# santurini/vsrlab

Hardware: AMD Instinct MI355X
Metric: LR frames/sec fwd+bwd, BasicVSR 4x 540p 7-frame clip, 1->8 MI355X (higher is better)
Workload: dtype bf16; 1 GPU; BasicVSR(mid=64,res_blocks=30,x4) fwd+Charbonnier+bwd+clip+Adam, 540x960->2160x3840, 7-frame clip, 2 clips per GPU (BASELINE configs[1]); clips_per_gpu=2, frames=7, res_blocks=30, parallelism=single GPU, arena=full, train_flow=False, trunk_chains=True

## Files before the change

### include/vsrlab_hip.h

```cpp
#ifndef VSRLAB_HIP_H
#define VSRLAB_HIP_H
#include <stddef.h>
#ifdef __cplusplus
extern "C" {
#endif

#define VSR_DT_F32 0
#define VSR_DT_BF16 1

#define VSR_STATUS_OK 0
#define VSR_STATUS_BADARG (-1)
#define VSR_STATUS_UNSUPPORTED (-2)
#define VSR_STATUS_HIP (-3)
#define VSR_STATUS_WORKSPACE (-4)

int vsr_abi_version(void);
const char* vsr_status_string(int status);

typedef struct VsrBasicVSRDesc {
    int n, t, h, w;
    int mid_channels;
    int res_blocks;
    int upscale;
    int dtype;
// ... 59 lines not shown

int vsr_flow_warp_fwd_ex(int dtype, const void* in_pm, const float* flow, void* out_pm, int N, int H, int W, int C,
                         int padding_mode, void* stream);
int vsr_flow_warp_bwd_ex(int dtype, const void* dout_pm, const float* flow, float* dacc_pm_f32, int N, int H, int W, int C,
                         int padding_mode, void* stream);
int vsr_flow_warp_bwd_flow_ex(int dtype, const void* in_pm, const void* dout_pm, const float* flow, float* dflow, int N,
                              int H, int W, int C, int padding_mode, void* stream);

int vsr_planar_to_pm(int dtype, const float* in, void* out_pm, int N, int Cin, int H, int W, int C,
                     void* stream);
int vsr_pm_to_planar(int dtype, const void* in_pm, float* out, int N, int Cout, int H, int W, int C,
                     void* stream);

int vsr_conv3x3_c64_fwd(int dtype, const void* x_pm, const float* w, const float* b, void* wpack,
                        void* y_pm, const void* res_pm, int act, int N, int H, int W, void* stream);

size_t vsr_conv3x3_c64_chain_sync_bytes(int nlayers, int N, int H, int W);
int vsr_conv3x3_c64_chain_fwd(const void* images, const void* wpack, const float* bias, int nlayers, int N, int H, int W,
                              void* sync, void* stream);
int vsr_conv3x3_c64_dgrad(int dtype, const void* dy_pm, const float* w, void* wpack, void* dx_pm,
                          const void* res_pm, const void* aux_pm, int mask_mode, int N, int H,
                          int W, void* stream);
int vsr_conv_layer_fwd(int dtype, int ks, const void* x_pm, int cin_pm, const float* lr_planar, const float* w,
                       const float* b, int cin_real, int cout_real, void* wpack, void* y_pm, int cd, float* y_planar,
                       int act, float slope, int pixel_shuffle, int N, int H, int W, void* stream);
size_t vsr_conv_layer_bwd_scratch_bytes(int dtype, int N, int H, int W, int pixel_shuffle);
int vsr_conv_layer_bwd(int dtype, int ks, const void* x_pm, int cin_pm, const float* lr_planar, const float* w, int cin_real,
                       int cout_real, const void* y_pm, const float* y_planar, const void* dy_pm, const float* dy_planar, int cd,
                       int act, float slope, int pixel_shuffle, void* dx_pm, float* dlr_planar, float* gw, float* gb,
                       void* scratch, size_t scratch_bytes, int N, int H, int W, void* stream);
size_t vsr_conv3x3_c64_wgrad_slab_floats(void);
int vsr_conv3x3_c64_wgrad(int dtype, const void* x_pm, const void* dy_pm, float* gw, float* gb,
                          float* slab, int N, int H, int W, void* stream);

size_t vsr_charbonnier_scratch_floats(void);
int vsr_charbonnier_fwd_bwd(const float* sr, const float* hr, float* dsr, float* loss, float* scratch, long long numel,
                            float eps, void* stream);

size_t vsr_optim_scratch_floats(void);
int vsr_adam_clip_step(float* params, const float* grads, float* exp_avg, float* exp_avg_sq, long long numel,
                       float lr, float beta1, float beta2, float eps, float weight_decay, int step, float grad_scale,
                       float max_norm, float* scratch, float* norm_out, void* stream);
int vsr_grad_norm(const float* grads, long long numel, float grad_scale, float* scratch, float* norm_out, void* stream);

int vsr_resize_bilinear(const float* in, float* out, long long planes, int H, int W, int h, int w, void* stream);

typedef struct VsrDiscDesc { int n, h, w, mid_ch, dtype; } VsrDiscDesc;
size_t vsr_disc_workspace_bytes(const VsrDiscDesc* d, int need_backward);
int vsr_disc_forward(const VsrDiscDesc* d, const float* const* params, int nparams, const float* img, float* out,
                     void* workspace, size_t workspace_bytes, int need_backward, void* stream);
int vsr_disc_backward(const VsrDiscDesc* d, float* const* grads, int nparams, const float* img, const float* dout,
                      float* dimg, void* workspace, size_t workspace_bytes, void* stream);

int vsr_spectral_norm(const float* w_orig, float* u, float* v, float* w_out, float* sigma, int rows, int cols,
                      int training, void* stream);
#define VSR_SN_SCRATCH_FLOATS 1024
int vsr_spectral_norm_backward(const float* dw, const float* w_orig, const float* u, const float* v, const float* sigma,
                               float* dw_orig, int rows, int cols, float* scratch, void* stream);

int vsr_bce_with_logits(const float* x, float target, float* dx, float* loss, long long numel, void* stream);

typedef struct VsrAttnDesc {
    int B, N, heads, head_dim;
    int q0, k0, o0, Nq, Nk;
    int Cout, c_off;
    int nW, Nm;
// ... 18 lines not shown
```

### vsrlab_amd/_lib.py

```python
import ctypes
import os
from ctypes import c_char_p, c_float, c_int, c_longlong, c_size_t, c_void_p

_HERE = os.path.dirname(os.path.abspath(__file__))
LIB_PATH = os.environ.get("VSRLAB_AMD_LIB") or os.path.join(_HERE, "lib", "libvsrlab_hip.so")

DT_F32 = 0
DT_BF16 = 1


class BasicVSRDesc(ctypes.Structure):
    _fields_ = [("n", c_int), ("t", c_int), ("h", c_int), ("w", c_int), ("mid_channels", c_int),
                ("res_blocks", c_int), ("upscale", c_int), ("dtype", c_int), ("arena_mode", c_int)]


class DiscDesc(ctypes.Structure):
    _fields_ = [("n", c_int), ("h", c_int), ("w", c_int), ("mid_ch", c_int), ("dtype", c_int)]


class AttnDesc(ctypes.Structure):
    _fields_ = [(k, c_int) for k in ("B", "N", "heads", "head_dim", "q0", "k0", "o0", "Nq", "Nk", "Cout", "c_off", "nW", "Nm")] + \
               [("scale", c_float), ("dtype", c_int), ("mask_packed", c_int), ("mask_value", c_float)]


# ... 7 lines not shown
    "vsr_basicvsr_backward": (c_int, [ctypes.POINTER(BasicVSRDesc), _P, _P, c_int, _P, _P, _P, _P, c_size_t, _P]),
    "vsr_basicvsr_get_flows": (c_int, [ctypes.POINTER(BasicVSRDesc), _P, _P, _P, _P]),
    "vsr_basicvsr_narrow_workspace_bytes": (c_size_t, [ctypes.POINTER(BasicVSRDesc), c_int]),
    "vsr_basicvsr_narrow_forward": (c_int, [ctypes.POINTER(BasicVSRDesc), _P, c_int, _P, _P, _P, c_size_t, c_int, _P]),
    "vsr_basicvsr_narrow_backward": (c_int, [ctypes.POINTER(BasicVSRDesc), _P, _P, c_int, _P, _P, _P, _P, c_size_t, _P]),
    "vsr_basicvsr_narrow_get_flows": (c_int, [ctypes.POINTER(BasicVSRDesc), _P, _P, _P, _P]),
    "vsr_spynet_workspace_bytes": (c_size_t, [c_int, c_int, c_int, c_int, c_int]),
    "vsr_spynet_forward": (c_int, [c_int, c_int, c_int, c_int, _P, c_int, _P, _P, _P, _P, c_size_t, c_int, _P]),
    "vsr_spynet_backward": (c_int, [c_int, c_int, c_int, c_int, _P, c_int, _P, _P, c_size_t, _P]),
    "vsr_spynet_forward_ex": (c_int, [c_int, c_int, c_int, c_int, _P, c_int, _P, _P, c_int, _P, _P, c_size_t, c_int, _P]),
    "vsr_spynet_backward_ex": (c_int, [c_int, c_int, c_int, c_int, _P, _P, c_int, _P, c_int, _P, _P, _P, _P, c_size_t, _P]),
    "vsr_cleaner_workspace_bytes": (c_size_t, [c_int, c_int, c_int, c_int, c_int, c_int, c_int]),
    "vsr_cleaner_narrow_workspace_bytes": (c_size_t, [c_int, c_int, c_int, c_int, c_int, c_int, c_int, c_int]),
    "vsr_cleaner_forward": (c_int, [c_int, c_int, c_int, c_int, c_int, c_int, c_int, _P, c_int, _P, _P, _P, c_size_t, c_int, _P]),
    "vsr_cleaner_backward": (c_int, [c_int, c_int, c_int, c_int, c_int, c_int, c_int, _P, c_int, _P, _P, _P, _P, c_size_t, _P]),
    "vsr_flow_warp_fwd": (c_int, [c_int, _P, _P, _P, c_int, c_int, c_int, c_int, _P]),
    "vsr_flow_warp_bwd": (c_int, [c_int, _P, _P, _P, c_int, c_int, c_int, c_int, _P]),
    "vsr_flow_warp_bwd_flow": (c_int, [c_int, _P, _P, _P, _P, c_int, c_int, c_int, c_int, _P]),
    "vsr_flow_warp_fwd_ex": (c_int, [c_int, _P, _P, _P, c_int, c_int, c_int, c_int, c_int, _P]),
    "vsr_flow_warp_bwd_ex": (c_int, [c_int, _P, _P, _P, c_int, c_int, c_int, c_int, c_int, _P]),
    "vsr_flow_warp_bwd_flow_ex": (c_int, [c_int, _P, _P, _P, _P, c_int, c_int, c_int, c_int, c_int, _P]),
    "vsr_planar_to_pm": (c_int, [c_int, _P, _P, c_int, c_int, c_int, c_int, c_int, _P]),
    "vsr_pm_to_planar": (c_int, [c_int, _P, _P, c_int, c_int, c_int, c_int, c_int, _P]),
    "vsr_conv3x3_c64_fwd": (c_int, [c_int, _P, _P, _P, _P, _P, _P, c_int, c_int, c_int, c_int, _P]),
    "vsr_conv3x3_c64_chain_sync_bytes": (c_size_t, [c_int, c_int, c_int, c_int]),
    "vsr_conv3x3_c64_chain_fwd": (c_int, [_P, _P, _P, c_int, c_int, c_int, c_int, _P, _P]),
    "vsr_conv3x3_c64_dgrad": (c_int, [c_int, _P, _P, _P, _P, _P, _P, c_int, c_int, c_int, c_int, _P]),
    "vsr_conv_layer_fwd": (c_int, [c_int, c_int, _P, c_int, _P, _P, _P, c_int, c_int, _P, _P, c_int, _P, c_int, c_float, c_int, c_int, c_int, c_int, _P]),
    "vsr_conv_layer_bwd_scratch_bytes": (c_size_t, [c_int, c_int, c_int, c_int, c_int]),
    "vsr_conv_layer_bwd": (c_int, [c_int, c_int, _P, c_int, _P, _P, c_int, c_int, _P, _P, _P, _P, c_int, c_int, c_float, c_int, _P, _P, _P, _P,
                                   _P, c_size_t, c_int, c_int, c_int, _P]),
    "vsr_conv3x3_c64_wgrad_slab_floats": (c_size_t, []),
    "vsr_conv3x3_c64_wgrad": (c_int, [c_int, _P, _P, _P, _P, _P, c_int, c_int, c_int, _P]),
    "vsr_charbonnier_scratch_floats": (c_size_t, []),
    "vsr_charbonnier_fwd_bwd": (c_int, [_P, _P, _P, _P, _P, c_longlong, c_float, _P]),
    "vsr_optim_scratch_floats": (c_size_t, []),
    "vsr_adam_clip_step": (c_int, [_P, _P, _P, _P, c_longlong, c_float, c_float, c_float, c_float, c_float, c_int, c_float,
                                   c_float, _P, _P, _P]),
    "vsr_grad_norm": (c_int, [_P, c_longlong, c_float, _P, _P, _P]),
    "vsr_resize_bilinear": (c_int, [_P, _P, c_longlong, c_int, c_int, c_int, c_int, _P]),
    "vsr_disc_workspace_bytes": (c_size_t, [ctypes.POINTER(DiscDesc), c_int]),
    "vsr_disc_forward": (c_int, [ctypes.POINTER(DiscDesc), _P, c_int, _P, _P, _P, c_size_t, c_int, _P]),
    "vsr_disc_backward": (c_int, [ctypes.POINTER(DiscDesc), _P, c_int, _P, _P, _P, _P, c_size_t, _P]),
    "vsr_spectral_norm": (c_int, [_P, _P, _P, _P, _P, c_int, c_int, c_int, _P]),
    "vsr_spectral_norm_backward": (c_int, [_P, _P, _P, _P, _P, _P, c_int, c_int, _P, _P]),
    "vsr_bce_with_logits": (c_int, [_P, c_float, _P, _P, c_longlong, _P]),
    "vsr_window_attention_fwd": (c_int, [ctypes.POINTER(AttnDesc), _P, _P, _P, _P, _P, _P]),
    "vsr_window_attention_bwd": (c_int, [ctypes.POINTER(AttnDesc), _P, _P, _P, _P, _P, _P, _P, _P, _P]),
    "vsr_mask_pack": (c_int, [_P, _P, c_int, c_int, _P]),
    "vsr_rpb_gather": (c_int, [_P, _P, c_int, _P, c_int, c_int, _P]),
    "vsr_rpb_scatter": (c_int, [_P, _P, c_int, _P, c_int, c_int, _P]),
}
EXPORTS = tuple(_SIGNATURES)

_lib = None


def load():
    global _lib
    if _lib is None:
        if not os.path.exists(LIB_PATH):
            raise RuntimeError(
                f"vsrlab_amd: HIP library not built ({LIB_PATH} missing). Run "
                "`python -c 'import __graft_entry__ as g; g.build()'` or `make -C vsrlab_amd/csrc`.")
        lib = ctypes.CDLL(LIB_PATH)
        for name, (res, args) in _SIGNATURES.items():
# ... 12 lines not shown
```

### vsrlab_amd/csrc/engine.hip

```cpp
#include <vector>
#include "kernels.h"
#include "../../include/vsrlab_hip.h"

namespace {

struct Bump {
    size_t off = 0;
    size_t take(size_t bytes) {
        size_t o = off;
        off += (bytes + 255) & ~size_t(255);
        return o;
    }
};

inline size_t esize(int dtype) { return dtype == VSR_BF16 ? 2 : 4; }

constexpr int C = 64;
constexpr int NSPY = 5;
const int SPY_CI[NSPY] = {8, 32, 64, 32, 16}, SPY_CO[NSPY] = {32, 64, 32, 16, 2};
const int SPY_CIP[NSPY] = {16, 32, 64, 32, 16}, SPY_COP[NSPY] = {32, 64, 32, 32, 32};
const int SPY_CD[NSPY] = {32, 64, 32, 16, 0};
const int SPY_DK[NSPY] = {32, 64, 32, 16, 16}, SPY_DROWS[NSPY] = {32, 32, 64, 32, 32};

struct SpyPlan {
// ... 589 lines not shown
    for (int k = 0; k < t; ++k) {
        const int i = dir == 0 ? t - 1 - k : k;
        void* warped = nullptr;
        if (k > 0) {
            const int prev = dir == 0 ? i + 1 : i - 1;
            warped = p.bwd ? c.at(p.Wp[dir][i]) : c.at(p.scratchW[dir]);
            CK(vsr_launch_warp_fwd(c.dtype, c.at(p.feat[dir][prev]), flow_ptr(c, p, dir, dir == 0 ? i : i - 1), warped, n, h, w, p.C, fstride, c.st));
        }
        CK(trunk_forward(c, p, dir, i, warped, lrs));
    }
    return VSR_OK;
}

int forward_impl(const Plan& p, const float* const* prm, const float* lrs, float* sr, char* ws, hipStream_t st) {
    const Ctx c{p, ws, st, p.dtype, 0};
    const PIdx ix{p.rb, p.ups};
    const int n = p.n, t = p.t;
    CK(pack_all(c, p, prm));
    if (t > 1) CK(spynet_run(c, p.spy, lrs, prm[ix.spy_mean()], prm[ix.spy_std()], n, t, 0, (float*)c.at(p.flows)));
    {
        Fork f{st, nullptr};
        CK(f.begin(!chain_on(p)));
        const Ctx c0{p, ws, st, p.dtype, 0}, c1{p, ws, f.side(), p.dtype, 1};
        CK(forward_chain(c0, p, 0, lrs));
        CK(forward_chain(c1, p, 1, lrs));
        CK(f.end());
    }
    for (int i = 0; i < t; ++i) CK(recon_forward(c, p, i, lrs, sr));
    return VSR_OK;
}

struct WG {
    const Ctx& c;
    int run(int ks, int cx, bool xp, int cout, bool dyp, WgradArgs& a, int cout_real, int cin_real, float* gw, int I_total,
            int i_off, int o_mul, int o_add, float* gb) const {
        if (!gw && !gb) return VSR_OK;
        int cp, xpd, stride;
        vsr_wgrad_slab_dims(ks, cx, cout, &cp, &xpd, &stride);
        a.slab = (float*)c.at(c.p.slab[c.lane]); a.slab_stride = stride;
        const int tiles = a.N * cdiv(a.H, 8) * cdiv(a.W, 32);
        int cp3, xp3, stride3;
        vsr_wgrad_slab_dims(3, 64, 64, &cp3, &xp3, &stride3);
        const long long cap = (long long)VSR_WGRAD_NWG * stride3 / stride;
        int nwg = tiles < VSR_WGRAD_NWG ? tiles : VSR_WGRAD_NWG;
        if (nwg > cap) nwg = (int)cap;
        if (nwg > 1) nwg &= ~1;
        int nslabs = 0;
        if (c.dtype == VSR_BF16 && ks == 3 && cx == 64 && !xp && cout == 16 && dyp && a.nseg == 1 && a.x_step == 1 && a.dy_step == 1 &&
            a.Hx == a.H && a.Wx == a.W && a.Hy == a.H && a.Wy == a.W) {
            CK(vsr_launch_last2_wgrad(a.x[0], reinterpret_cast<const float*>(a.dy[0]), a.dy_nstride, a.slab, stride, a.N, a.H, a.W, &nslabs, c.st));
        } else
        CK(vsr_launch_wgrad(c.dtype, ks, cx, xp, cout, dyp, a, nwg, &nslabs, c.st));
        if (!gw) return VSR_ERR_BADARG;
        return vsr_launch_wgrad_reduce(a.slab, nslabs, ks, cx, cout, cout_real, cin_real, gw, I_total, i_off, o_mul, o_add, gb, 1, c.st);
    }
};

WgradArgs wg_base(int N, int H, int W, int Cx = C, int Cy = C) {
    WgradArgs a = {};
    a.N = N; a.H = H; a.W = W; a.nseg = 1;
    a.x_step = 1; a.Hx = H; a.Wx = W; a.x_nstride = pm_image_elems(H, W, Cx);
    a.dy_step = 1; a.Hy = H; a.Wy = W; a.dy_nstride = pm_image_elems(H, W, Cy);
    return a;
}

int spynet_backward(const Ctx& c, const SpyPlan& sp, const float* dflows_out, int n, int t, int pair_mode, float* const* g,
                    int base_idx, float* dframes = nullptr, const float* std = nullptr, bool last_relu = true,
                    const float* const* dlevel = nullptr) {
    const WG wg{c};
    const int P = sp.P, hu = sp.hu, wu = sp.wu;
    size_t dcur = sp.dfa, dprev = sp.dfb;
    HIP_CHECK_RET(hipMemsetAsync(c.at(dcur), 0, (size_t)P * 2 * hu * wu * 4, c.st));
    if (dflows_out) CK(vsr_launch_flow_out_bwd(dflows_out, (float*)c.at(dcur), P, hu, wu, sp.h, sp.w, c.st));
    if (dframes)
        for (int l = 0; l < 6; ++l)
            HIP_CHECK_RET(hipMemsetAsync(c.at(sp.dpyr[l]), 0, (size_t)sp.F * 3 * (hu >> (5 - l)) * (wu >> (5 - l)) * 4, c.st));
    for (int l = 5; l >= 0; --l) {
        const int hl = hu >> (5 - l), wl = wu >> (5 - l);
        if (dlevel && dlevel[l])
// ... 42 lines not shown
        CK(vsr_launch_resize_norm_bwd(c.fat(sp.dpyr[5]), dframes, std, sp.F, sp.h, sp.w, hu, wu, c.st));
    }
    return VSR_OK;
}

int recon_ps_wgrads(const Ctx& c, const Plan& p, int k, int f0, int f1, float* const* g) {
    const PIdx ix{p.rb, p.ups};
    const WG wg{c};
    const int n = p.n, H = (k + 1) * p.h, W = (k + 1) * p.w;
    const int C = p.C;
    for (int i0 = f0; i0 < f1; i0 += VSR_WG_MAXSEG) {
        const int i1 = i0 + VSR_WG_MAXSEG < f1 ? i0 + VSR_WG_MAXSEG : f1;
        for (int z = 0; z < 4; ++z) {
            WgradArgs a = wg_base(n, H, W, C, C);
            a.nseg = 0;
            for (int i = i0; i < i1; ++i) {
                a.x[a.nseg] = c.at(k == 1 ? p.U0[i] : p.Pt[i]);
                const char* gu = (const char*)c.at(k == 1 ? p.GU1f[i] : p.GU0f[i]);
                a.dy[a.nseg] = p.unsh ? gu + (size_t)z * Ctx::plane_elems(n, 2 * H, 2 * W) * p.es : gu;
                ++a.nseg;
            }
            if (!p.unsh) { a.dy_step = 2; a.dy_oy = z >> 1; a.dy_ox = z & 1; a.Hy = 2 * H; a.Wy = 2 * W; a.dy_nstride = pm_image_elems(2 * H, 2 * W, C); }
            CK(wg.run(3, C, false, C, false, a, C, C, g[ix.up_w(k)], C, 0, 4, z, g[ix.up_b(k)]));
        }
    }
    return VSR_OK;
}
int recon_point_wgrads(const Ctx& c, const Plan& p, int f0, int f1, float* const* g) {
    const PIdx ix{p.rb, p.ups};
    const WG wg{c};
    const int C = p.C;
    for (int i0 = f0; i0 < f1; i0 += VSR_WG_MAXSEG) {
        const int i1 = i0 + VSR_WG_MAXSEG < f1 ? i0 + VSR_WG_MAXSEG : f1;
        for (int s = 0; s < 2; ++s) {
            WgradArgs a = wg_base(p.n, p.h, p.w, C, C);
            a.nseg = 0;
            for (int i = i0; i < i1; ++i) { a.x[a.nseg] = c.at(p.feat[s][i]); a.dy[a.nseg] = c.at(p.GPf[i]); ++a.nseg; }
            CK(wg.run(1, C, false, C, false, a, C, C, g[ix.point_w()], 2 * C, s * C, 1, 0, s == 0 ? g[ix.point_b()] : nullptr));
        }
    }
    return VSR_OK;
}

int recon_backward(const Ctx& c, const Plan& p, int i, const float* lrs, const float* dsr, float* const* g, const float* last2_w) {
    const PIdx ix{p.rb, p.ups};
    const WG wg{c};
    if (p.diet) {
        CK(c.conv_ps(c.at(p.Pt[i]), p.up_w[0], c.fat(p.up_b[0]), c.at(p.U0[i]), p.n, p.h, p.w));
        if (p.ups == 2) CK(c.conv_ps(c.at(p.U0[i]), p.up_w[1], c.fat(p.up_b[1]), c.at(p.U1[i]), p.n, 2 * p.h, 2 * p.w));
        CK(last0_forward(c, p, i, nullptr));
    }
    const int C = p.C;
    const int n = p.n, h = p.h, w = p.w, H4 = p.scale * h, W4 = p.scale * w;
    const float* dsr_i = dsr + (size_t)i * 3 * H4 * W4;
    const long long dsr_ns = (long long)p.t * 3 * H4 * W4;
    if (c.dtype == VSR_BF16 && last2_w) {
        CK(vsr_launch_last2_dgrad(dsr_i, dsr_ns, last2_w, c.at(p.C0[i]), c.at(p.G_C0), n, H4, W4, MASK_LEAKY, c.st, p.sb ? c.at(p.SBC0[i]) : nullptr));
    } else {
        ConvArgs a = c.base(n, H4, W4);
        a.src[0] = dsr_i; a.src_nstride[0] = dsr_ns; a.wpack = c.at(p.last2_wd); a.dst[0] = c.at(p.G_C0);
        a.aux[0] = c.at(p.C0[i]); a.mask_mode = MASK_LEAKY;
        a.CD = 64; a.cout_real = 64; a.dst_nstride = pm_image_elems(H4, W4, 64);
        CK(vsr_launch_conv(c.dtype, 3, 1, 16, 16, 1, 64, EPI_NHWC, a, c.st));
    }
    {
        WgradArgs a = wg_base(n, H4, W4, 64, 64);
// ... 37 lines not shown
    if (pending_flow) {
        const long long fstride = (long long)(p.t - 1) * 2 * h * w;
        CK(vsr_launch_warp_bwd_gather(c.dtype, c.at(p.dWp[dir]), pending_flow, dtop, (long long*)c.at(p.S[dir]),
                                      (int*)c.at(p.far_cnt) + dir * 32 + pending_k, c.at(p.dxoff(dir, i, rb)), n, h, w, p.C, fstride, c.st));
    } else {
        CK(vsr_launch_add_cast(c.dtype, dtop, nullptr, c.at(p.dxoff(dir, i, rb)), n, h, w, p.C, c.st));
    }
    const bool chain = chain_on(p) && !p.diet;
    if (chain) CK(trunk_chain_backward(c, p, dir, i));
    for (int b = chain ? 0 : rb - 1; b >= 0; --b) {
        const void* dxn = c.at(p.dxoff(dir, i, b + 1));
        if (!chain) CK(c.conv64(dxn, p.blk_wd[dir][2 * b + 1], nullptr, c.at(p.g1off(dir, i, b)), ACT_NONE, nullptr, c.at(p.aoff(dir, i, b)), MASK_RELU, n, h, w,
                    nullptr, p.sb ? c.at(p.sboff(dir, i, b)) : nullptr));
        void* out = b > 0 ? c.at(p.dxoff(dir, i, b)) : c.at(p.G0[dir][i]);
        CK(c.conv64(c.at(p.g1off(dir, i, b)), p.blk_wd[dir][2 * b], nullptr, out, ACT_NONE, dxn, b == 0 ? c.at(p.xoff(dir, i, 0)) : nullptr,
                    b == 0 ? MASK_LEAKY : 0, n, h, w, nullptr, (b == 0 && p.sb) ? c.at(p.SBX0[dir][i]) : nullptr));
        if (p.diet) CK(block_wgrads(c, p, dir, b, i, i + 1, g));
    }
    if (has_warp)
        CK(c.conv64(c.at(p.G0[dir][i]), p.stem_wd[dir], nullptr, c.at(p.dWp[dir]), ACT_NONE, nullptr, nullptr, 0, n, h, w));
    if (p.diet) CK(stem_wgrads(c, p, dir, i, i + 1, lrs, g));
    return VSR_OK;
}

int stem_wgrads(const Ctx& c, const Plan& p, int dir, int f0, int f1, const float* lrs, float* const* g) {
    const PIdx ix{p.rb, p.ups};
    const WG wg{c};
    const int n = p.n, t = p.t, h = p.h, w = p.w, C = p.C;
    {
        WgradArgs a = wg_base(n, h, w, C, C);
        a.nseg = 0;
        for (int i = f0; i < f1; ++i) { a.x[a.nseg] = lrs + (size_t)i * 3 * h * w; a.dy[a.nseg] = c.at(p.G0[dir][i]); ++a.nseg; }
        a.x_nstride = (long long)t * 3 * h * w;
        CK(wg.run(3, 16, true, C, false, a, C, 3, g[ix.stem_w(dir)], C + 3, 0, 1, 0, g[ix.stem_b(dir)]));
    }
    {
        WgradArgs a = wg_base(n, h, w, C, C);
        a.nseg = 0;
        for (int i = f0; i < f1; ++i) {
            const bool has = dir == 0 ? (i < t - 1) : (i > 0);
            if (has) { a.x[a.nseg] = c.at(p.Wp[dir][i]); a.dy[a.nseg] = c.at(p.G0[dir][i]); ++a.nseg; }
        }
        if (a.nseg) CK(wg.run(3, C, false, C, false, a, C, C, g[ix.stem_w(dir)], C + 3, 3, 1, 0, nullptr));
    }
    return VSR_OK;
}
int block_wgrads(const Ctx& c, const Plan& p, int dir, int b, int f0, int f1, float* const* g) {
    const PIdx ix{p.rb, p.ups};
    const WG wg{c};
    const int C = p.C;
    WgradArgs a1 = wg_base(p.n, p.h, p.w, C, C), a2 = wg_base(p.n, p.h, p.w, C, C);
    a1.nseg = a2.nseg = 0;
    for (int i = f0; i < f1; ++i) {
        a1.x[a1.nseg] = c.at(p.xoff(dir, i, b)); a1.dy[a1.nseg] = c.at(p.g1off(dir, i, b)); ++a1.nseg;
        a2.x[a2.nseg] = c.at(p.aoff(dir, i, b)); a2.dy[a2.nseg] = c.at(p.dxoff(dir, i, b + 1)); ++a2.nseg;
    }
    CK(wg.run(3, C, false, C, false, a1, C, C, g[ix.blk_w(dir, 2 * b)], C, 0, 1, 0, g[ix.blk_b(dir, 2 * b)]));
    CK(wg.run(3, C, false, C, false, a2, C, C, g[ix.blk_w(dir, 2 * b + 1)], C, 0, 1, 0, g[ix.blk_b(dir, 2 * b + 1)]));
    return VSR_OK;
}
int trunk_wgrads(const Ctx& c, const Plan& p, int dir, const float* lrs, float* const* g) {
    for (int i0 = 0; i0 < p.t; i0 += VSR_WG_MAXSEG) {
        const int i1 = i0 + VSR_WG_MAXSEG < p.t ? i0 + VSR_WG_MAXSEG : p.t;
        CK(stem_wgrads(c, p, dir, i0, i1, lrs, g));
        for (int b = 0; b < p.rb; ++b) CK(block_wgrads(c, p, dir, b, i0, i1, g));
    }
    return VSR_OK;
// ... 742 lines not shown
            if (!y_pm || cd != SPY_CD[j]) return VSR_ERR_BADARG;
            a.dst[0] = y_pm; a.CD = SPY_CD[j]; a.dst_nstride = pm_image_elems(H, W, SPY_CD[j]);
            return vsr_launch_conv(dtype, 7, 1, SPY_CIP[j], SPY_CIP[j], 0, SPY_COP[j], EPI_NHWC, a, st);
        }
        if (!y_planar) return VSR_ERR_BADARG;
        a.dst[0] = y_planar; a.dst_nstride = (long long)2 * H * W;
        return vsr_launch_conv(dtype, 7, 1, 16, 16, 0, 32, EPI_PLANAR, a, st);
    }
    return VSR_ERR_UNSUPPORTED;
}

size_t vsr_conv3x3_c64_wgrad_slab_floats(void) {
    int cp, xp, stride;
    vsr_wgrad_slab_dims(3, 64, 64, &cp, &xp, &stride);
    return (size_t)VSR_WGRAD_NWG * stride;
}

int vsr_conv3x3_c64_wgrad(int dtype, const void* x_pm, const void* dy_pm, float* gw, float* gb, float* slab, int N, int H, int W,
                          void* stream) {
    if (bad_dtype(dtype) || !x_pm || !dy_pm || !gw || !slab || bad_dims(N, H, W)) return VSR_ERR_BADARG;
    hipStream_t st = (hipStream_t)stream;
    WgradArgs a = wg_base(N, H, W);
    a.x[0] = x_pm; a.dy[0] = dy_pm;
    int cp, xp, stride;
    vsr_wgrad_slab_dims(3, 64, 64, &cp, &xp, &stride);
    a.slab = slab; a.slab_stride = stride;
    const int tiles = N * cdiv(H, 8) * cdiv(W, 32);
    const int nwg = tiles < VSR_WGRAD_NWG ? tiles : VSR_WGRAD_NWG;
    int nslabs = 0;
    CK(vsr_launch_wgrad(dtype, 3, 64, 0, 64, 0, a, nwg, &nslabs, st));
    return vsr_launch_wgrad_reduce(slab, nslabs, 3, 64, 64, C, C, gw, C, 0, 1, 0, gb, 0, st);
}

size_t vsr_charbonnier_scratch_floats(void) { return (size_t)vsr_charbonnier_scratch_floats_impl(); }
int vsr_charbonnier_fwd_bwd(const float* sr, const float* hr, float* dsr, float* loss, float* scratch, long long numel, float eps, void* stream) {
    if (!sr || !hr || !dsr || !loss || !scratch || numel < 1) return VSR_ERR_BADARG;
    return vsr_launch_charbonnier_grad(sr, hr, dsr, loss, scratch, numel, eps, (hipStream_t)stream);
}

}
```

### vsrlab_amd/csrc/kernels.h

```cpp
#pragma once
#include "common.h"

int vsr_launch_conv(int dtype, int ks, int nsrc, int ca, int cb, int last_planar, int cout_t, int epi,
                    const ConvArgs& a, hipStream_t st);
int vsr_launch_sign_bits_c64(const void* x_pm, void* bits, int N, int H, int W, hipStream_t st);

enum { CHAIN_RELU = 0,
       CHAIN_SKIP = 1,
       CHAIN_MASK = 2 };
#define VSR_CHAIN_MAX_LAYERS 64
struct ChainLayer { unsigned src, dst, res, sbits, sout, w, bias; int variant; };
struct ChainArgs {
    char* base;
    unsigned* sync;
    int N, H, W, nlayers;
    ChainLayer layer[VSR_CHAIN_MAX_LAYERS];
};
size_t vsr_chain_sync_bytes(int nlayers, int N, int H, int W);
int vsr_launch_conv3x3_chain(const ChainArgs& a, int num_cus, hipStream_t st);
void vsr_wgrad_slab_dims(int ks, int cx, int cout, int* coutp, int* cxp, int* stride);
int vsr_launch_wgrad(int dtype, int ks, int cx, int x_planar, int cout, int dy_planar, const WgradArgs& a, int nwg,
                     int* nslabs, hipStream_t st);
int vsr_launch_wgrad_reduce(const float* slab, int nwg, int ks, int cx, int cout, int cout_real, int cin_real, float* gw,
                            int I_total, int i_off, int o_mul, int o_add, float* gb, int accumulate, hipStream_t st);
int vsr_launch_warp_fwd(int dtype, const void* in, const float* flow, void* out, int N, int H, int W, int C,
                        long long flow_nstride, hipStream_t st, int border = 0);
int vsr_launch_warp_bwd(int dtype, const void* dout, const float* flow, float* dacc, int N, int H, int W, int C,
                        long long flow_nstride, hipStream_t st, int border = 0);
int vsr_launch_warp_bwd_gather(int dtype, const void* dout, const float* flow, const void* dtop, long long* S, int* far_count, void* out,
                               int N, int H, int W, int C, long long flow_nstride, hipStream_t st);
int vsr_launch_add_cast(int dtype, const void* a, const float* s, void* out, int N, int H, int W, int C, hipStream_t st);
int vsr_launch_planar_to_pm(int dtype, const float* in, void* out, int N, int Cin, int H, int W, int C, hipStream_t st);
int vsr_launch_pm_to_planar(int dtype, const void* in, float* out, int N, int Cout, int H, int W, int C, hipStream_t st);
int vsr_launch_resize_norm(const float* in, float* out, const float* mean, const float* std, int F, int h, int w, int hu,
                           int wu, hipStream_t st);
int vsr_launch_avgpool2(const float* in, float* out, long long planes, int h, int w, hipStream_t st);
int vsr_launch_spynet_prepare(int dtype, const float* frames, const float* flow_prev, float* flow_up, void* x16, int n,
                              int t, int P, int pair_mode, int h, int w, int level0, hipStream_t st);
int vsr_launch_flow_out(const float* in, float* out, int P, int hu, int wu, int h, int w, hipStream_t st);
int vsr_launch_warp_bwd_flow(int dtype, const void* in, const void* dout, const float* flow, float* dflow, int N, int H, int W,
                             int C, long long flow_nstride, hipStream_t st, int border = 0);
int vsr_launch_spynet_dres(int dtype, const float* dflow, const float* res, void* out, int P, int h, int w, hipStream_t st);
int vsr_launch_spynet_prepare_bwd(int dtype, const void* dx16, const float* dflow_l, const float* frames, const float* flow_up,
                                  float* dflow_prev, float* dframes, int n, int t, int P, int pair_mode, int h, int w, hipStream_t st);
int vsr_launch_avgpool2_bwd_add(const float* dcoarse, float* dfine, long long planes, int h, int w, hipStream_t st);
int vsr_launch_resize_norm_bwd(const float* dnorm, float* dframes, const float* std, int F, int h, int w, int hu, int wu, hipStream_t st);
int vsr_launch_bilinear4_bwd(const float* dsr, float* dlr, long long planes, int h, int w, hipStream_t st, int scale = 4);
int vsr_launch_flow_out_bwd(const float* dout, float* din, int P, int hu, int wu, int h, int w, hipStream_t st);
int vsr_launch_add_f32(const float* a, const float* b, float* out, long long n, hipStream_t st);
int vsr_launch_c64_to_planar(const ConvArgs& a, hipStream_t st);
int vsr_launch_last2_wgrad(const void* x, const float* dy, long long dy_nstride, float* slab, int slab_stride, int N, int H, int W,
                           int* nslabs, hipStream_t st, int pc = 3);
int vsr_launch_last2_dgrad(const float* dsr, long long dsr_nstride, const float* w, const void* aux, void* dst, int N, int H, int W,
                           int mask_mode, hipStream_t st, const void* sign_bits = nullptr, float slope = 0.f);
struct VsrPackDesc {
    const float* w; void* dst;
    int total, blk0;
// ... 35 lines not shown
```

### vsrlab_amd/csrc/wgrad_mfma.hip

```cpp
#include <cstdlib>
#include "kernels.h"

namespace {

constexpr int TW = 32, TH = 8, NTHREADS = 256;

template <typename T> struct WElt;
template <> struct WElt<bf16_t> { static constexpr int CHB = 16; typedef uint4 chunk_t; };
struct wchunk32_t { uint4 a, b; };
template <> struct WElt<float> { static constexpr int CHB = 32; typedef wchunk32_t chunk_t; };

template <typename T> __device__ __forceinline__ typename WElt<T>::chunk_t wzero();
template <> __device__ __forceinline__ uint4 wzero<bf16_t>() { return make_uint4(0, 0, 0, 0); }
template <> __device__ __forceinline__ wchunk32_t wzero<float>() { wchunk32_t z; z.a = make_uint4(0, 0, 0, 0); z.b = z.a; return z; }

__device__ __forceinline__ uint4 wchunk3(float a, float b, float c, bf16_t*) {
    union { bf16_t h[8]; uint4 u; } t; t.u = make_uint4(0, 0, 0, 0);
    t.h[0] = (bf16_t)a; t.h[1] = (bf16_t)b; t.h[2] = (bf16_t)c; return t.u;
}
__device__ __forceinline__ wchunk32_t wchunk3(float a, float b, float c, float*) {
    wchunk32_t t; t.a = make_uint4(__float_as_uint(a), __float_as_uint(b), __float_as_uint(c), 0); t.b = make_uint4(0, 0, 0, 0); return t;
}
__device__ __forceinline__ void chunk_sum(const uint4& v, float* s) {
    union { uint4 u; bf16_t h[8]; } t; t.u = v;
// ... 567 lines not shown
                        slab[((long long)t * 64 + cb * 32 + m * 16 + 4 * q + j) * 64 + ib * 32 + n * 16 + l15] = acc[t][m][n][j];
        __syncthreads();
        __syncthreads();
        if (tid < 64) {
            const float* red = reinterpret_cast<const float*>(smem);
            float s = 0.f;
            const int c = tid >> 3, j = tid & 7;
            for (int t = c; t < 256; t += 8) s += red[t * 8 + j];
            slab[9 * 64 * 64 + tid] = s;
        }
    }
#ifdef VSR_ABL
    if (tid == 0 && blockIdx.x < 256) {
        g_wclk[blockIdx.x * 4 + 0] = __builtin_amdgcn_s_memtime() - clk_t0;
        g_wclk[blockIdx.x * 4 + 1] = __builtin_amdgcn_s_memrealtime() - clk_r0;
        g_wclk[blockIdx.x * 4 + 2] = clk_bar;
        g_wclk[blockIdx.x * 4 + 3] = clk_tiles;
    }
#endif
}

int launch_wgrad_pc(const WgradArgs& a0, int nwg, hipStream_t st) {
    constexpr int LDS = 2 * DSET;
    static VsrDevOnce once;
    { const int rc = vsr_set_max_dynamic_lds(once, reinterpret_cast<const void*>(wgrad3x3_c64_pc_kernel), LDS); if (rc != VSR_OK) return rc; }
    WgradArgs a = a0;
    a.ntiles_x = cdiv(a.W, TW);
    a.ntiles_y = cdiv(a.H, TH);
    hipLaunchKernelGGL(wgrad3x3_c64_pc_kernel, dim3(nwg), dim3(DNT), LDS, st, a);
    HIP_CHECK_RET(hipGetLastError());
    return VSR_OK;
}

}

#ifdef VSR_ABL
extern "C" int vsr_debug_read_wclk(unsigned long long* host_out) {
    return hipMemcpyFromSymbol(host_out, HIP_SYMBOL(g_wclk), sizeof(unsigned long long) * 256 * 4) == hipSuccess ? 0 : -3;
}
#endif



#define VSR_WGRAD_SHAPES(X)           \
    X(3, 64, false, 64, false)         \
    X(3, 16, true, 64, false)          \
    X(3, 64, false, 16, true)          \
    X(1, 64, false, 64, false)         \
    X(7, 16, false, 32, false)         \
    X(7, 32, false, 64, false)         \
    X(7, 64, false, 32, false)         \
    X(7, 32, false, 32, false)        \
    X(7, 32, false, 16, false)         \
    X(7, 16, false, 16, false)         \
     \
    X(3, 16, false, 16, false)         \
    X(3, 32, false, 32, false)         \
    X(3, 16, true, 16, false)          \
    X(3, 16, true, 32, false)          \
    X(1, 16, false, 16, false)         \
    X(1, 32, false, 32, false)        \
    X(3, 16, false, 64, false)         \
    X(3, 32, false, 64, false)        \
    X(3, 16, false, 16, true)          \
    X(3, 32, false, 16, true)

// ... 78 lines not shown
```

Before: 56.83 LR frames/s.

## Add specialized MFMA wgrad kernels for 128-ch pointwise fuse and LR stem conv

Adds a point_wgrad2 kernel that computes the 1x1 fusion-conv weight gradient over both 64-channel input halves in a single pass, sharing the dy tile instead of launching the generic wgrad twice. Also adds a stem_lr_wgrad kernel that reads the planar fp32 LR frames directly with a halo tile and runs 3x3x3 taps as a bf16 MFMA, replacing the padded 16-channel generic path. Both kernels fall back to the generic wgrad when shapes or dtype are unsupported. This reduces redundant dy reads and wasted padded-channel MFMA work, at the cost of more specialized code and a larger LDS footprint.

```diff
diff --git a/include/vsrlab_hip.h b/include/vsrlab_hip.h
--- a/include/vsrlab_hip.h
+++ b/include/vsrlab_hip.h
@@ -115,6 +115,10 @@
 size_t vsr_conv3x3_c64_wgrad_slab_floats(void);
 int vsr_conv3x3_c64_wgrad(int dtype, const void* x_pm, const void* dy_pm, float* gw, float* gb,
                           float* slab, int N, int H, int W, void* stream);
+int vsr_point_conv_wgrad(int dtype, const void* const* x0_pm, const void* const* x1_pm, const void* const* dy_pm, int nseg,
+                         float* gw, float* gb, float* slab, int N, int H, int W, int generic, void* stream);
+int vsr_stem_lr_wgrad(int dtype, const float* const* lr_planar, long long lr_nstride, const void* const* dy_pm, int nseg, float* gw,
+                      float* gb, float* slab, int N, int H, int W, int generic, void* stream);
 
 size_t vsr_charbonnier_scratch_floats(void);
 int vsr_charbonnier_fwd_bwd(const float* sr, const float* hr, float* dsr, float* loss, float* scratch, long long numel,
diff --git a/vsrlab_amd/_lib.py b/vsrlab_amd/_lib.py
--- a/vsrlab_amd/_lib.py
+++ b/vsrlab_amd/_lib.py
@@ -63,6 +63,8 @@
                                    _P, c_size_t, c_int, c_int, c_int, _P]),
     "vsr_conv3x3_c64_wgrad_slab_floats": (c_size_t, []),
     "vsr_conv3x3_c64_wgrad": (c_int, [c_int, _P, _P, _P, _P, _P, c_int, c_int, c_int, _P]),
+    "vsr_point_conv_wgrad": (c_int, [c_int, _P, _P, _P, c_int, _P, _P, _P, c_int, c_int, c_int, c_int, _P]),
+    "vsr_stem_lr_wgrad": (c_int, [c_int, _P, c_longlong, _P, c_int, _P, _P, _P, c_int, c_int, c_int, c_int, _P]),
     "vsr_charbonnier_scratch_floats": (c_size_t, []),
     "vsr_charbonnier_fwd_bwd": (c_int, [_P, _P, _P, _P, _P, c_longlong, c_float, _P]),
     "vsr_optim_scratch_floats": (c_size_t, []),
diff --git a/vsrlab_amd/csrc/engine.hip b/vsrlab_amd/csrc/engine.hip
--- a/vsrlab_amd/csrc/engine.hip
+++ b/vsrlab_amd/csrc/engine.hip
@@ -645,11 +645,7 @@
 
 struct WG {
     const Ctx& c;
-    int run(int ks, int cx, bool xp, int cout, bool dyp, WgradArgs& a, int cout_real, int cin_real, float* gw, int I_total,
-            int i_off, int o_mul, int o_add, float* gb) const {
-        if (!gw && !gb) return VSR_OK;
-        int cp, xpd, stride;
-        vsr_wgrad_slab_dims(ks, cx, cout, &cp, &xpd, &stride);
+    int slab_nwg(WgradArgs& a, int stride) const {
         a.slab = (float*)c.at(c.p.slab[c.lane]); a.slab_stride = stride;
         const int tiles = a.N * cdiv(a.H, 8) * cdiv(a.W, 32);
         int cp3, xp3, stride3;
@@ -658,6 +654,34 @@
         int nwg = tiles < VSR_WGRAD_NWG ? tiles : VSR_WGRAD_NWG;
         if (nwg > cap) nwg = (int)cap;
         if (nwg > 1) nwg &= ~1;
+        return nwg;
+    }
+    int run_point2(WgradArgs& a, const void* const* x1, float* gw, float* gb) const {
+        if (!gw) return gb ? VSR_ERR_BADARG : VSR_OK;
+        int cp, xpd, stride;
+        vsr_wgrad_slab_dims(1, 128, 64, &cp, &xpd, &stride);
+        const int nwg = slab_nwg(a, stride);
+        int nslabs = 0;
+        const int rc = vsr_launch_point_wgrad2(c.dtype, a, x1, nwg, &nslabs, c.st);
+        if (rc != VSR_OK) return rc;
+        return vsr_launch_wgrad_reduce(a.slab, nslabs, 1, 128, 64, 64, 128, gw, 128, 0, 1, 0, gb, 1, c.st);
+    }
+    int run_stem_lr(WgradArgs& a, float* gw, float* gb) const {
+        if (!gw) return gb ? VSR_ERR_BADARG : VSR_OK;
+        int cp, xpd, stride;
+        vsr_wgrad_slab_dims(3, 16, 64, &cp, &xpd, &stride);
+        const int nwg = slab_nwg(a, stride);
+        int nslabs = 0;
+        const int rc = vsr_launch_stem_lr_wgrad(c.dtype, a, nwg, &nslabs, c.st);
+        if (rc != VSR_OK) return rc;
+        return vsr_launch_wgrad_reduce(a.slab, nslabs, 3, 16, 64, 64, 3, gw, 64 + 3, 0, 1, 0, gb, 1, c.st);
+    }
+    int run(int ks, int cx, bool xp, int cout, bool dyp, WgradArgs& a, int cout_real, int cin_real, float* gw, int I_total,
+            int i_off, int o_mul, int o_add, float* gb) const {
+        if (!gw && !gb) return VSR_OK;
+        int cp, xpd, stride;
+        vsr_wgrad_slab_dims(ks, cx, cout, &cp, &xpd, &stride);
+        const int nwg = slab_nwg(a, stride);
         int nslabs = 0;
         if (c.dtype == VSR_BF16 && ks == 3 && cx == 64 && !xp && cout == 16 && dyp && a.nseg == 1 && a.x_step == 1 && a.dy_step == 1 &&
             a.Hx == a.H && a.Wx == a.W && a.Hy == a.H && a.Wy == a.W) {
@@ -766,6 +790,15 @@
     const int C = p.C;
     for (int i0 = f0; i0 < f1; i0 += VSR_WG_MAXSEG) {
         const int i1 = i0 + VSR_WG_MAXSEG < f1 ? i0 + VSR_WG_MAXSEG : f1;
+        if (C == 64) {
+            WgradArgs a = wg_base(p.n, p.h, p.w, C, C);
+            const void* x1[VSR_WG_MAXSEG];
+            a.nseg = 0;
+            for (int i = i0; i < i1; ++i) { a.x[a.nseg] = c.at(p.feat[0][i]); x1[a.nseg] = c.at(p.feat[1][i]); a.dy[a.nseg] = c.at(p.GPf[i]); ++a.nseg; }
+            const int rc = wg.run_point2(a, x1, g[ix.point_w()], g[ix.point_b()]);
+            if (rc == VSR_OK) continue;
+            if (rc != VSR_ERR_UNSUPPORTED) return rc;
+        }
         for (int s = 0; s < 2; ++s) {
             WgradArgs a = wg_base(p.n, p.h, p.w, C, C);
             a.nseg = 0;
@@ -869,7 +902,9 @@
         a.nseg = 0;
         for (int i = f0; i < f1; ++i) { a.x[a.nseg] = lrs + (size_t)i * 3 * h * w; a.dy[a.nseg] = c.at(p.G0[dir][i]); ++a.nseg; }
         a.x_nstride = (long long)t * 3 * h * w;
-        CK(wg.run(3, 16, true, C, false, a, C, 3, g[ix.stem_w(dir)], C + 3, 0, 1, 0, g[ix.stem_b(dir)]));
+        const int rc = C == 64 ? wg.run_stem_lr(a, g[ix.stem_w(dir)], g[ix.stem_b(dir)]) : VSR_ERR_UNSUPPORTED;
+        if (rc != VSR_ERR_UNSUPPORTED) CK(rc);
+        else CK(wg.run(3, 16, true, C, false, a, C, 3, g[ix.stem_w(dir)], C + 3, 0, 1, 0, g[ix.stem_b(dir)]));
     }
     {
         WgradArgs a = wg_base(n, h, w, C, C);
@@ -1678,6 +1713,63 @@
     return vsr_launch_wgrad_reduce(slab, nslabs, 3, 64, 64, C, C, gw, C, 0, 1, 0, gb, 0, st);
 }
 
+int vsr_point_conv_wgrad(int dtype, const void* const* x0_pm, const void* const* x1_pm, const void* const* dy_pm, int nseg,
+                         float* gw, float* gb, float* slab, int N, int H, int W, int generic, void* stream) {
+    if (bad_dtype(dtype) || !x0_pm || !x1_pm || !dy_pm || nseg < 1 || nseg > VSR_WG_MAXSEG || !gw || !slab || bad_dims(N, H, W)) return VSR_ERR_BADARG;
+    hipStream_t st = (hipStream_t)stream;
+    WgradArgs a = wg_base(N, H, W);
+    a.nseg = nseg;
+    for (int s = 0; s < nseg; ++s) {
+        if (!x0_pm[s] || !x1_pm[s] || !dy_pm[s]) return VSR_ERR_BADARG;
+        a.x[s] = x0_pm[s]; a.dy[s] = dy_pm[s];
+    }
+    a.slab = slab;
+    const int tiles = N * cdiv(H, 8) * cdiv(W, 32);
+    int nwg = tiles < VSR_WGRAD_NWG ? tiles : VSR_WGRAD_NWG;
+    if (nwg > 1) nwg &= ~1;
+    int cp, xp, stride, nslabs = 0;
+    if (!generic) {
+        vsr_wgrad_slab_dims(1, 128, 64, &cp, &xp, &stride);
+        a.slab_stride = stride;
+        const int rc = vsr_launch_point_wgrad2(dtype, a, x1_pm, nwg, &nslabs, st);
+        if (rc == VSR_OK) return vsr_launch_wgrad_reduce(slab, nslabs, 1, 128, 64, 64, 128, gw, 128, 0, 1, 0, gb, 0, st);
+        if (rc != VSR_ERR_UNSUPPORTED) return rc;
+    }
+    vsr_wgrad_slab_dims(1, 64, 64, &cp, &xp, &stride);
+    a.slab_stride = stride;
+    for (int h = 0; h < 2; ++h) {
+        if (h) for (int s = 0; s < nseg; ++s) a.x[s] = x1_pm[s];
+        CK(vsr_launch_wgrad(dtype, 1, 64, 0, 64, 0, a, nwg, &nslabs, st));
+        CK(vsr_launch_wgrad_reduce(slab, nslabs, 1, 64, 64, 64, 64, gw, 128, h * 64, 1, 0, h ? nullptr : gb, 0, st));
+    }
+    return VSR_OK;
+}
+
+int vsr_stem_lr_wgrad(int dtype, const float* const* lr_planar, long long lr_nstride, const void* const* dy_pm, int nseg, float* gw, float* gb,
+                      float* slab, int N, int H, int W, int generic, void* stream) {
+    if (bad_dtype(dtype) || !lr_planar || !dy_pm || nseg < 1 || nseg > VSR_WG_MAXSEG || !gw || !slab || bad_dims(N, H, W) ||
+        lr_nstride < 3LL * H * W) return VSR_ERR_BADARG;
+    hipStream_t st = (hipStream_t)stream;
+    WgradArgs a = wg_base(N, H, W);
+    a.nseg = nseg;
+    a.x_nstride = lr_nstride;
+    for (int s = 0; s < nseg; ++s) {
+        if (!lr_planar[s] || !dy_pm[s]) return VSR_ERR_BADARG;
+        a.x[s] = lr_planar[s]; a.dy[s] = dy_pm[s];
+    }
+    a.slab = slab;
+    const int tiles = N * cdiv(H, 8) * cdiv(W, 32);
+    int nwg = tiles < VSR_WGRAD_NWG ? tiles : VSR_WGRAD_NWG;
+    if (nwg > 1) nwg &= ~1;
+    int cp, xp, stride, nslabs = 0;
+    vsr_wgrad_slab_dims(3, 16, 64, &cp, &xp, &stride);
+    a.slab_stride = stride;
+    int rc = generic ? VSR_ERR_UNSUPPORTED : vsr_launch_stem_lr_wgrad(dtype, a, nwg, &nslabs, st);
+    if (rc == VSR_ERR_UNSUPPORTED) rc = vsr_launch_wgrad(dtype, 3, 16, 1, 64, 0, a, nwg, &nslabs, st);
+    CK(rc);
+    return vsr_launch_wgrad_reduce(slab, nslabs, 3, 16, 64, 64, 3, gw, 3, 0, 1, 0, gb, 0, st);
+}
+
 size_t vsr_charbonnier_scratch_floats(void) { return (size_t)vsr_charbonnier_scratch_floats_impl(); }
 int vsr_charbonnier_fwd_bwd(const float* sr, const float* hr, float* dsr, float* loss, float* scratch, long long numel, float eps, void* stream) {
     if (!sr || !hr || !dsr || !loss || !scratch || numel < 1) return VSR_ERR_BADARG;
diff --git a/vsrlab_amd/csrc/kernels.h b/vsrlab_amd/csrc/kernels.h
--- a/vsrlab_amd/csrc/kernels.h
+++ b/vsrlab_amd/csrc/kernels.h
@@ -23,6 +23,8 @@
                      int* nslabs, hipStream_t st);
 int vsr_launch_wgrad_reduce(const float* slab, int nwg, int ks, int cx, int cout, int cout_real, int cin_real, float* gw,
                             int I_total, int i_off, int o_mul, int o_add, float* gb, int accumulate, hipStream_t st);
+int vsr_launch_point_wgrad2(int dtype, const WgradArgs& a, const void* const* x1, int nwg, int* nslabs, hipStream_t st);
+int vsr_launch_stem_lr_wgrad(int dtype, const WgradArgs& a, int nwg, int* nslabs, hipStream_t st);
 int vsr_launch_warp_fwd(int dtype, const void* in, const float* flow, void* out, int N, int H, int W, int C,
                         long long flow_nstride, hipStream_t st, int border = 0);
 int vsr_launch_warp_bwd(int dtype, const void* dout, const float* flow, float* dacc, int N, int H, int W, int C,
diff --git a/vsrlab_amd/csrc/wgrad_mfma.hip b/vsrlab_amd/csrc/wgrad_mfma.hip
--- a/vsrlab_amd/csrc/wgrad_mfma.hip
+++ b/vsrlab_amd/csrc/wgrad_mfma.hip
@@ -623,6 +623,285 @@
     return VSR_OK;
 }
 
+struct WgPtrs { const void* p[VSR_WG_MAXSEG]; };
+constexpr int PW_NT = 512;
+constexpr int PW_TB = TH * TW * 8 * 16;
+__global__ __launch_bounds__(PW_NT, 1) void point_wgrad2_kernel(const WgradArgs a, const WgPtrs x1) {
+    extern __shared__ __attribute__((aligned(16))) char smem[];
+    char* ly = smem;
+    const int tid = threadIdx.x, lane = tid & 63, wave = tid >> 6;
+    const int l31 = lane & 31, h = lane >> 5;
+    const int cb = wave & 1, ib = wave >> 1;
+    const bool ystager = tid < 256;
+    const int tiles_per_img = a.ntiles_x * a.ntiles_y;
+    const int ntiles = a.N * tiles_per_img;
+    const uint4* zsrc = g_wg_zero;
+
+    f32x16_t acc;
+#pragma unroll
+    for (int j = 0; j < 16; ++j) acc[j] = 0.f;
+    float bsum[8];
+#pragma unroll
+    for (int j = 0; j < 8; ++j) bsum[j] = 0.f;
+
+    const int xe0 = ystager ? tid : 1024 + (tid - 256);
+    uint4 v[12];
+    auto load = [&](int seg, int tile) {
+        const int n = tile / tiles_per_img, tr = tile - n * tiles_per_img;
+        const int ty0 = (tr / a.ntiles_x) * TH, tx0 = (tr % a.ntiles_x) * TW;
+        const bf16_t* xb0 = reinterpret_cast<const bf16_t*>(a.x[seg]) + (long long)n * a.x_nstride;
+        const bf16_t* xb1 = reinterpret_cast<const bf16_t*>(x1.p[seg]) + (long long)n * a.x_nstride;
+        auto ldx = [&](int ex) {
+            const int idx = ex & 2047, p = idx >> 3, c = idx & 7;
+            const int vy = ty0 + p / TW, vx = tx0 + (p & (TW - 1));
+            const bool in = vy < a.H && vx < a.W;
+            return *(in ? reinterpret_cast<const uint4*>(((ex >> 11) ? xb1 : xb0) + pm_off(vy, vx, c, a.W, 64)) : zsrc);
+        };
+        if (ystager) {
+            const bf16_t* yb = reinterpret_cast<const bf16_t*>(a.dy[seg]) + (long long)n * a.dy_nstride;
+#pragma unroll
+            for (int k = 0; k < 8; ++k) {
+                const int idx = tid + 256 * k, p = idx >> 3, c = idx & 7;
+                const int vy = ty0 + p / TW, vx = tx0 + (p & (TW - 1));
+                const bool in = vy < a.H && vx < a.W;
+                v[k] = *(in ? reinterpret_cast<const uint4*>(yb + pm_off(vy, vx, c, a.W, 64)) : zsrc);
+            }
+#pragma unroll
+            for (int k = 0; k < 4; ++k) v[8 + k] = ldx(xe0 + 256 * k);
+        } else {
+#pragma unroll
+            for (int k = 0; k < 12; ++k) v[k] = ldx(xe0 + 256 * k);
+        }
+    };
+    auto stx = [&](int ex, const uint4& val) {
+        const int idx = ex & 2047, p = idx >> 3, c = idx & 7;
+        *reinterpret_cast<uint4*>(ly + PW_TB * (1 + (ex >> 11)) + (p * 8 + wswz<8>(p, c)) * 16) = val;
+    };
+    auto store = [&]() {
+        if (ystager) {
+#pragma unroll
+            for (int k = 0; k < 8; ++k) {
+                const int idx = tid + 256 * k, p = idx >> 3, c = idx & 7;
+                chunk_sum(v[k], bsum);
+                *reinterpret_cast<uint4*>(ly + (p * 8 + wswz<8>(p, c)) * 16) = v[k];
+            }
+#pragma unroll
+            for (int k = 0; k < 4; ++k) stx(xe0 + 256 * k, v[8 + k]);
+        } else {
+#pragma unroll
+            for (int k = 0; k < 12; ++k) stx(xe0 + 256 * k, v[k]);
+        }
+    };
+
+    int seg = 0, tile = blockIdx.x;
+    if (a.nseg > 0) load(seg, tile);
+    const char* lx = smem + PW_TB * (1 + (ib >> 1));
+    const int g2 = (lane >> 4) & 1, q = (lane & 15) >> 2, p4 = (lane & 3) * 4;
+    const int chy = cb * 32 + 16 * g2 + p4, chx = (ib & 1) * 32 + 16 * g2 + p4;
+    while (seg < a.nseg) {
+        __syncthreads();
+        store();
+        __syncthreads();
+        tile += gridDim.x;
+        if (tile >= ntiles) { tile = blockIdx.x; ++seg; }
+        if (seg < a.nseg) load(seg, tile);
+        for (int row = 0; row < TH; ++row) {
+#pragma unroll
+            for (int half = 0; half < 2; ++half) {
+                const int py = row * TW + half * 16 + 8 * h + q;
+                const s16x4_t a0 = tr_read(ly + lds_addr<bf16_t, 8>(py, chy));
+                const s16x4_t a1 = tr_read(ly + lds_addr<bf16_t, 8>(py + 4, chy));
+                const s16x4_t b0 = tr_read(lx + lds_addr<bf16_t, 8>(py, chx));
+                const s16x4_t b1 = tr_read(lx + lds_addr<bf16_t, 8>(py + 4, chx));
+                union { s16x4_t s[2]; bf16x8_t b; } ua, ub;
+                ua.s[0] = a0; ua.s[1] = a1; ub.s[0] = b0; ub.s[1] = b1;
+                acc = __builtin_amdgcn_mfma_f32_32x32x16_bf16(ua.b, ub.b, acc, 0, 0, 0);
+            }
+        }
+    }
+
+    float* slab = a.slab + (long long)blockIdx.x * a.slab_stride;
+#pragma unroll
+    for (int r = 0; r < 16; ++r) {
+        const int co = cb * 32 + (r & 3) + 8 * (r >> 2) + 4 * h;
+        slab[(long long)co * 128 + ib * 32 + l31] = acc[r];
+    }
+    __syncthreads();
+    float* red = reinterpret_cast<float*>(smem);
+    if (ystager) {
+#pragma unroll
+        for (int j = 0; j < 8; ++j) red[tid * 8 + j] = bsum[j];
+    }
+    __syncthreads();
+    if (tid < 64) {
+        const int c = tid >> 3, j = tid & 7;
+        float s = 0.f;
+        for (int t = c; t < 256; t += 8) s += red[t * 8 + j];
+        slab[64 * 128 + tid] = s;
+    }
+}
+
+constexpr int SL_RS = TW + 2, SL_PL = (TH + 2) * SL_RS;
+constexpr int SL_YB = TH * TW * 8 * 16;
+__global__ __launch_bounds__(NTHREADS, 2) void stem_lr_wgrad_kernel(const WgradArgs a) {
+    extern __shared__ __attribute__((aligned(16))) char smem[];
+    char* ly = smem;
+    float* lt = reinterpret_cast<float*>(smem + SL_YB);
+    const int tid = threadIdx.x, lane = tid & 63, wave = tid >> 6;
+    const int l31 = lane & 31, h = lane >> 5;
+    const int tiles_per_img = a.ntiles_x * a.ntiles_y;
+    const int ntiles = a.N * tiles_per_img;
+    const long long plane = (long long)a.Hx * a.Wx;
+    const uint4* zsrc = g_wg_zero;
+    const float* zf = reinterpret_cast<const float*>(g_wg_zero);
+
+    f32x16_t acc[2];
+#pragma unroll
+    for (int m = 0; m < 2; ++m)
+#pragma unroll
+        for (int j = 0; j < 16; ++j) acc[m][j] = 0.f;
+    float bsum[8];
+#pragma unroll
+    for (int j = 0; j < 8; ++j) bsum[j] = 0.f;
+
+    uint4 v[8];
+    float f[4];
+    auto load = [&](int seg, int tile) {
+        const int n = tile / tiles_per_img, tr = tile - n * tiles_per_img;
+        const int ty0 = (tr / a.ntiles_x) * TH, tx0 = (tr % a.ntiles_x) * TW;
+        const bf16_t* yb = reinterpret_cast<const bf16_t*>(a.dy[seg]) + (long long)n * a.dy_nstride;
+#pragma unroll
+        for (int k = 0; k < 8; ++k) {
+            const int idx = tid + NTHREADS * k, p = idx >> 3, c = idx & 7;
+            const int vy = ty0 + p / TW, vx = tx0 + (p & (TW - 1));
+            const bool in = vy < a.H && vx < a.W;
+            v[k] = *(in ? reinterpret_cast<const uint4*>(yb + pm_off(vy, vx, c, a.W, 64)) : zsrc);
+        }
+        const float* xb = reinterpret_cast<const float*>(a.x[seg]) + (long long)n * a.x_nstride;
+#pragma unroll
+        for (int k = 0; k < 4; ++k) {
+            const int e = tid + NTHREADS * k;
+            const int c = e / SL_PL, rem = e - c * SL_PL, yy = rem / SL_RS, xx = rem - yy * SL_RS;
+            const int vy = ty0 + yy - 1, vx = tx0 + xx - 1;
+            const bool in = e < 3 * SL_PL && vy >= 0 && vy < a.H && vx >= 0 && vx < a.W;
+            f[k] = *(in ? xb + c * plane + (long long)vy * a.Wx + vx : zf);
+        }
+    };
+    auto store = [&]() {
+#pragma unroll
+        for (int k = 0; k < 8; ++k) {
+            const int idx = tid + NTHREADS * k, p = idx >> 3, c = idx & 7;
+            chunk_sum(v[k], bsum);
+            *reinterpret_cast<uint4*>(ly + (p * 8 + wswz<8>(p, c)) * 16) = v[k];
+        }
+#pragma unroll
+        for (int k = 0; k < 4; ++k) lt[tid + NTHREADS * k] = f[k];
+    };
+
+    const int tap = l31 / 3, ci = l31 - 3 * tap, ky = tap / 3, kx = tap - 3 * ky;
+    const bool bcol = l31 < 27;
+    const int boff = bcol ? ci * SL_PL + ky * SL_RS + kx + 8 * h : 0;
+    const int g2 = (lane >> 4) & 1, q = (lane & 15) >> 2, p4 = (lane & 3) * 4;
+
+    int seg = 0, tile = blockIdx.x;
+    if (a.nseg > 0) load(seg, tile);
+    while (seg < a.nseg) {
+        __syncthreads();
+        store();
+        __syncthreads();
+        tile += gridDim.x;
+        if (tile >= ntiles) { tile = blockIdx.x; ++seg; }
+        if (seg < a.nseg) load(seg, tile);
+#pragma unroll
+        for (int rr = 0; rr < 2; ++rr) {
+            const int row = 2 * wave + rr;
+#pragma unroll
+            for (int half = 0; half < 2; ++half) {
+                const int xk = half * 16;
+                bf16x8_t fb;
+                const float* bp = lt + boff + row * SL_RS + xk;
+#pragma unroll
+                for (int j = 0; j < 8; ++j) fb[j] = (bf16_t)(bcol ? bp[j] : 0.f);
+                const int py = row * TW + xk + 8 * h + q;
+#pragma unroll
+                for (int cb = 0; cb < 2; ++cb) {
+                    const int chy = cb * 32 + 16 * g2 + p4;
+                    union { s16x4_t s[2]; bf16x8_t b; } ua;
+                    ua.s[0] = tr_read(ly + lds_addr<bf16_t, 8>(py, chy));
+                    ua.s[1] = tr_read(ly + lds_addr<bf16_t, 8>(py + 4, chy));
+                    acc[cb] = __builtin_amdgcn_mfma_f32_32x32x16_bf16(ua.b, fb, acc[cb], 0, 0, 0);
+                }
+            }
+        }
+    }
+
+    float* slab = a.slab + (long long)blockIdx.x * a.slab_stride;
+    float* red = reinterpret_cast<float*>(smem);
+    __syncthreads();
+#pragma unroll
+    for (int cb = 0; cb < 2; ++cb)
+#pragma unroll
+        for (int r = 0; r < 16; ++r) {
+            const int co = cb * 32 + (r & 3) + 8 * (r >> 2) + 4 * h;
+            red[(wave * 64 + co) * 32 + l31] = acc[cb][r];
+        }
+    __syncthreads();
+    for (int e = tid; e < 64 * 27; e += NTHREADS) {
+        const int co = e / 27, n = e - co * 27, t = n / 3, c = n - 3 * t;
+        const float s = (red[co * 32 + n] + red[(64 + co) * 32 + n]) + (red[(128 + co) * 32 + n] + red[(192 + co) * 32 + n]);
+        slab[((long long)t * 64 + co) * 32 + c] = s;
+    }
+    __syncthreads();
+#pragma unroll
+    for (int j = 0; j < 8; ++j) red[tid * 8 + j] = bsum[j];
+    __syncthreads();
+    if (tid < 64) {
+        const int c = tid >> 3, j = tid & 7;
+        float s = 0.f;
+        for (int t = c; t < NTHREADS; t += 8) s += red[t * 8 + j];
+        slab[9 * 64 * 32 + tid] = s;
+    }
+}
+
+}
+
+int vsr_launch_stem_lr_wgrad(int dtype, const WgradArgs& a0, int nwg, int* nslabs, hipStream_t st) {
+    if (a0.nseg < 1 || a0.nseg > VSR_WG_MAXSEG || nwg < 1 || !nslabs) return VSR_ERR_BADARG;
+    if (dtype != VSR_BF16 || vsr_env().generic_wgrad || a0.x_step != 1 || a0.dy_step != 1 || a0.x_oy || a0.x_ox || a0.dy_oy || a0.dy_ox ||
+        a0.Hx != a0.H || a0.Wx != a0.W || a0.Hy != a0.H || a0.Wy != a0.W || a0.dy_ctotal || a0.dy_coff ||
+        a0.dy_nstride != pm_image_elems(a0.H, a0.W, 64) || a0.x_nstride < 3LL * a0.H * a0.W || nwg > a0.N * cdiv(a0.H, TH) * cdiv(a0.W, TW))
+        return VSR_ERR_UNSUPPORTED;
+    constexpr int LDS = SL_YB + 4 * NTHREADS * 4;
+    static VsrDevOnce once;
+    { const int rc = vsr_set_max_dynamic_lds(once, reinterpret_cast<const void*>(stem_lr_wgrad_kernel), LDS); if (rc != VSR_OK) return rc; }
+    WgradArgs a = a0;
+    a.ntiles_x = cdiv(a.W, TW);
+    a.ntiles_y = cdiv(a.H, TH);
+    hipLaunchKernelGGL(stem_lr_wgrad_kernel, dim3(nwg), dim3(NTHREADS), LDS, st, a);
+    HIP_CHECK_RET(hipGetLastError());
+    *nslabs = nwg;
+    return VSR_OK;
+}
+
+int vsr_launch_point_wgrad2(int dtype, const WgradArgs& a0, const void* const* x1, int nwg, int* nslabs, hipStream_t st) {
+    if (a0.nseg < 1 || a0.nseg > VSR_WG_MAXSEG || nwg < 1 || !nslabs || !x1) return VSR_ERR_BADARG;
+    if (dtype != VSR_BF16 || vsr_env().generic_wgrad || a0.x_step != 1 || a0.dy_step != 1 || a0.x_oy || a0.x_ox || a0.dy_oy || a0.dy_ox ||
+        a0.Hx != a0.H || a0.Wx != a0.W || a0.Hy != a0.H || a0.Wy != a0.W || a0.x_ctotal || a0.x_coff || a0.dy_ctotal || a0.dy_coff ||
+        a0.x_nstride != pm_image_elems(a0.H, a0.W, 64) || a0.dy_nstride != pm_image_elems(a0.H, a0.W, 64) ||
+        nwg > a0.N * cdiv(a0.H, TH) * cdiv(a0.W, TW))
+        return VSR_ERR_UNSUPPORTED;
+    constexpr int LDS = 3 * PW_TB;
+    static VsrDevOnce once;
+    { const int rc = vsr_set_max_dynamic_lds(once, reinterpret_cast<const void*>(point_wgrad2_kernel), LDS); if (rc != VSR_OK) return rc; }
+    WgradArgs a = a0;
+    a.ntiles_x = cdiv(a.W, TW);
+    a.ntiles_y = cdiv(a.H, TH);
+    WgPtrs p = {};
+    for (int s = 0; s < a.nseg; ++s) p.p[s] = x1[s];
+    hipLaunchKernelGGL(point_wgrad2_kernel, dim3(nwg), dim3(PW_NT), LDS, st, a, p);
+    HIP_CHECK_RET(hipGetLastError());
+    *nslabs = nwg;
+    return VSR_OK;
 }
 
 #ifdef VSR_ABL
```

After: 57.00 LR frames/s (median of 6 runs). Within noise of the previous version (+0.3%).
